# tau-dev/SdfBox

Measured on AMD Instinct MI355X. Metric: Mray/s (primary rays; frame W*H / time per frame), higher is better.
Workload: dtype f32

## Files before the change

### include/sdfhip_experimental.h

```cpp
#ifndef SDFHIP_EXPERIMENTAL_H
#define SDFHIP_EXPERIMENTAL_H

#include "sdfhip.h"

#ifdef __cplusplus
extern "C" {
#endif

enum {
    SDFHIP_FLAG_WIRE = 0x10000,
    SDFHIP_TUNE_ORDER_SHIFT = 8,
    SDFHIP_TUNE_BLOCK_SHIFT = 12,
    SDFHIP_TUNE_ONE_KERNEL = 0x20000,
    SDFHIP_TUNE_LDS_TOP = 0x40000,
    SDFHIP_TUNE_SHADOW_QUEUE = 0x80000,
    SDFHIP_TUNE_BYTE_CELLS = 0x200000,
    SDFHIP_TUNE_PERSISTENT_WAVES = 0x400000
};


SDFHIP_API int sdfhip_multi_debug_floats_sent(sdfhip_multi *m, uint32_t floats);

SDFHIP_API int sdfhip_debug_tile_order(sdfhip_scene *scene, const uint32_t *d_perm, uint16_t *d_cost);

SDFHIP_API int sdfhip_debug_touch_begin(sdfhip_scene *scene);
SDFHIP_API int sdfhip_debug_touch_end(sdfhip_scene *scene, uint64_t *out, uint32_t max_phases, uint32_t *n_phases, uint64_t *array_bytes4);

SDFHIP_API int sdfhip_debug_fail_host_allocations(int64_t countdown, uint64_t *thrown_so_far);

SDFHIP_API int sdfhip_debug_step_classes(sdfhip_scene *scene, void *stream, uint64_t *out6);

SDFHIP_API int sdfhip_debug_unorm_table(int device, float *out256);

#ifdef __cplusplus
}
#endif
#endif
```

### sdfbox_amd/_lib.py

```python
import ctypes
import os

_HERE = os.path.dirname(os.path.abspath(__file__))
LIB_PATH = os.path.abspath(os.environ.get("SDFHIP_LIB") or os.path.join(_HERE, "libsdfhip.so"))
LAB_LIB_PATH = os.path.join(_HERE, "libsdfhip_lab.so")

try:
    import torch
except Exception:
    torch = None

if not os.path.exists(LIB_PATH):
    raise ImportError(
        f"{LIB_PATH} is missing: build it with `make -C {os.path.join(_HERE, 'csrc')}` "
        "(hipcc --offload-arch=gfx950). sdfbox_amd has no CPU fallback.")

lib = ctypes.CDLL(LIB_PATH)

OK, ERR_ARG, ERR_IO, ERR_BAD_TREE, ERR_DEVICE, ERR_NOMEM = range(6)

KERNEL_AUTO, KERNEL_GENERIC, KERNEL_STACK = 0, 1, 2
FLAG_COMPACT, FLAG_COUNT, FLAG_DISPLAY, FLAG_DISPLAY_DEBUG = 0x10, 0x20, 0x40, 0x80
FLAG_TILE_ORDER = 0x100000
FLAG_WIRE = 0x10000
# ... 515 lines not shown
    "sdfhip_trimesh_prepare": (_c.c_int, [_vp, _c.c_uint32, _c.c_uint32, _c.POINTER(TriMeshOptions), _c.POINTER(CTriMesh)]),
    "sdfhip_trimesh_free": (None, [_c.POINTER(CTriMesh)]),
    "sdfhip_trimesh_build": (_c.c_int, [_c.c_int, _c.POINTER(CTriMesh), _c.c_int32, _c.POINTER(_vp), _c.POINTER(COctData),
                                        _c.POINTER(TriMeshStats)]),
    "sdfhip_scene_top_grid": (_c.c_int, [_vp, _c.POINTER(_c.c_int32), _c.POINTER(_c.c_uint64)]),
    "sdfhip_render_bands_device": (_c.c_int, [_vp, _c.POINTER(Info), _c.c_uint32, _c.POINTER(PathTrace), _c.c_uint32,
                                              _c.c_uint32, _c.c_uint32, _c.POINTER(_c.c_uint16), _c.c_uint32,
                                              _c.c_uint32, _c.c_uint32, _vp, _vp, _c.POINTER(Stats)]),
    "sdfhip_deinterleave_bands_device": (_c.c_int, [_c.c_int, _vp, _vp, _c.c_uint32, _c.c_uint32, _c.c_uint32,
                                                    _c.c_uint32, _c.c_uint32, _c.POINTER(_c.c_uint8), _c.c_uint32,
                                                    _c.c_uint32, _vp]),
    "sdfhip_sparse2_bytes": (_c.c_uint64, [_c.c_uint32, _c.c_uint32, _c.c_uint32, _c.c_uint32]),
    "sdfhip_sparse2_floats_offset": (_c.c_uint64, [_c.c_uint32, _c.c_uint32, _c.c_uint32]),
    "sdfhip_render_sparse_device": (_c.c_int, [_vp, _c.POINTER(Info), _c.c_uint32, _c.c_uint32, _c.c_uint32, _c.c_uint32,
                                               _c.POINTER(_c.c_uint16), _c.c_uint32, _c.c_uint32, _c.c_uint32, _c.c_uint32, _c.c_uint32, _vp, _vp]),
    "sdfhip_deinterleave_sparse2_device": (_c.c_int, [_c.c_int, _c.POINTER(_vp), _vp, _c.c_uint32, _c.c_uint32, _c.c_uint32,
                                                      _c.c_uint32, _c.c_uint32, _c.POINTER(_c.c_uint8), _c.c_uint32, _c.c_uint32,
                                                      _c.c_uint32, _c.c_int, _vp, _vp]),
    "sdfhip_multi_create": (_c.c_int, [_c.POINTER(_c.c_int), _c.c_uint32, _vp, _vp, _c.c_uint32, _c.POINTER(_vp)]),
    "sdfhip_multi_free": (_c.c_int, [_vp]),
    "sdfhip_multi_configure": (_c.c_int, [_vp, _c.c_uint32, _c.c_float]),
    "sdfhip_multi_info": (_c.c_int, [_vp, _c.POINTER(_c.c_uint32), _c.POINTER(_c.c_int), _c.POINTER(_c.c_uint32),
                                     _c.POINTER(_c.c_float), _c.POINTER(_c.c_int)]),
    "sdfhip_multi_render": (_c.c_int, [_vp, _c.POINTER(Info), _c.c_uint32, _c.c_uint32, _c.c_uint32, _vp, _c.POINTER(MultiStats)]),
    "sdfhip_multi_render_path": (_c.c_int, [_vp, _c.POINTER(Info), _c.POINTER(PathTrace), _c.c_uint32, _c.c_uint32, _c.c_uint32,
                                            _vp, _c.POINTER(MultiStats)]),
    "sdfhip_multi_submit": (_c.c_int, [_vp, _c.c_uint32, _c.POINTER(Info), _c.c_uint32, _c.c_uint32, _c.c_uint32, _c.c_uint32, _vp]),
    "sdfhip_multi_submit_path": (_c.c_int, [_vp, _c.c_uint32, _c.POINTER(Info), _c.POINTER(PathTrace), _c.c_uint32, _c.c_uint32,
                                            _c.c_uint32, _vp]),
    "sdfhip_multi_wait": (_c.c_int, [_vp, _c.c_uint32, _c.POINTER(_vp), _c.POINTER(MultiStats)]),
}
_SIG_LAB = {
    "sdfhip_debug_tile_order": (_c.c_int, [_vp, _vp, _vp]),
    "sdfhip_debug_unorm_table": (_c.c_int, [_c.c_int, _vp]),
    "sdfhip_debug_step_classes": (_c.c_int, [_vp, _vp, _c.POINTER(_c.c_uint64)]),
    "sdfhip_multi_debug_floats_sent": (_c.c_int, [_vp, _c.c_uint32]),
    "sdfhip_debug_fail_host_allocations": (_c.c_int, [_c.c_int64, _c.POINTER(_c.c_uint64)]),
    "sdfhip_debug_touch_begin": (_c.c_int, [_vp]),
    "sdfhip_debug_touch_end": (_c.c_int, [_vp, _c.POINTER(_c.c_uint64), _c.c_uint32, _c.POINTER(_c.c_uint32), _c.POINTER(_c.c_uint64)]),
}
for _name, (_res, _args) in _SIG.items():
    _fn = getattr(lib, _name)
    _fn.restype = _res
    _fn.argtypes = _args
EXPERIMENTS = hasattr(lib, "sdfhip_debug_unorm_table")
if EXPERIMENTS:
    for _name, (_res, _args) in _SIG_LAB.items():
        _fn = getattr(lib, _name)
        _fn.restype = _res
        _fn.argtypes = _args

EXPORTED_SYMBOLS = tuple(_SIG)
EXPERIMENTAL_SYMBOLS = tuple(_SIG_LAB)


def need_lab(what):
    if not EXPERIMENTS:
        raise RuntimeError(f"{what} is part of the experiments build (include/sdfhip_experimental.h): load libsdfhip_lab.so "
                           "(sdfbox_amd.lab.load(), or SDFHIP_LIB=sdfbox_amd/libsdfhip_lab.so)")



def check(code):
    if code != OK:
        raise SdfHipError(code, lib.sdfhip_last_error().decode("utf-8", "replace"))
```

### sdfbox_amd/csrc/lab.hip

```cpp
#ifndef SDFHIP_EXPERIMENTS
#error "lab.hip belongs to the experiments build (-DSDFHIP_EXPERIMENTS)"
#endif
#include "lab_kernels.h"
#include "scene.h"
#include "abi_guard.h"
#include "../../include/sdfhip_experimental.h"

#include <atomic>
#include <cstdlib>
#include <new>

using namespace sdfhip;

void sdfhip::build_dense4(sdfhip_scene *s)
{
    const int F = (int)s->depth;
    if (!s->stack_ok || !s->d_top || F < 1 || F > 10 || s->top_level + s->fine_bits != F) return;
    const char *env = getenv("SDFHIP_SAMPLE_RECORDS");
    if (!env || atoi(env) != 1) return;
    const size_t ncell = (size_t)1 << (3 * F);
    if (ncell * 4 > s->total_mem / 32) return;
    const GridRef g{s->d_top, s->d_fine, s->top_level, s->fine_bits, 0};
    const uint32_t n_chunks = (uint32_t)((ncell + 255) / 256);
    uint32_t *d4 = nullptr, *d_chunks = nullptr;
// ... 120 lines not shown
            if (cur == CUR_STACK_SPLIT) { if (count) go(k_path<CUR_STACK_SPLIT, true>); else go(k_path<CUR_STACK_SPLIT, false>); }
            else                        { if (count) go(k_path<CUR_STACK_FULL, true>); else go(k_path<CUR_STACK_FULL, false>); }
            *launched = true;
        }
        return SDFHIP_OK;
    }
    if (compact) return SDFHIP_OK;
    const uint32_t tile_w = bt >= 128 ? 16u : 8u, tile_h = (uint32_t)bt / 8u / (tile_w / 8u);
    P.tiles_x = (c.width + tile_w - 1) / tile_w;
    P.tiles_y = (c.nrows_out + tile_h - 1) / tile_h;
    P.n_tiles = P.tiles_x * P.tiles_y;
    const dim3 gp(P.tile_order == 0 ? 8u * ((P.tiles_y + 7u) / 8u) * P.tiles_x : P.n_tiles, c.n_frames);
    if ((flags & SDFHIP_TUNE_LDS_TOP) && cur == CUR_STACK && s->d_top && s->top_level <= 3 && !count) {
        if (bt == 256) hipLaunchKernelGGL((k_plain<CUR_STACK, false, 256, true>), gp, dim3(256), 0, st, P);
        else           hipLaunchKernelGGL((k_plain<CUR_STACK, false, 64, true>), gp, dim3(64), 0, st, P);
    }
    else if (cur == CUR_STACK_SPLIT) { if (count) launch_plain<CUR_STACK_SPLIT, true>(bt, gp, st, P); else launch_plain<CUR_STACK_SPLIT, false>(bt, gp, st, P); }
    else if (cur == CUR_STACK_FULL)  { if (count) launch_plain<CUR_STACK_FULL, true>(bt, gp, st, P); else launch_plain<CUR_STACK_FULL, false>(bt, gp, st, P); }
    else if (cur == CUR_STACK)       { if (count) launch_plain<CUR_STACK, true>(bt, gp, st, P); else launch_plain<CUR_STACK, false>(bt, gp, st, P); }
    else                             { if (count) launch_plain<CUR_GENERIC, true>(bt, gp, st, P); else launch_plain<CUR_GENERIC, false>(bt, gp, st, P); }
    *launched = true;
    return SDFHIP_OK;
}

extern "C" int sdfhip_debug_tile_order(sdfhip_scene *s, const uint32_t *d_perm, uint16_t *d_cost)
try {
    if (!s) return fail(SDFHIP_ERR_ARG, "debug_tile_order: null scene");
    std::lock_guard<std::mutex> lk(s->lock);
    s->dbg_tile_perm = d_perm; s->dbg_tile_cost = d_cost;
    return SDFHIP_OK;
}
SDFHIP_ABI_CATCH(sdfhip_debug_tile_order)

static void touch_release(sdfhip_scene *s)
{
    for (int a = 0; a < 4; a++) { if (s->touch.bits[a]) (void)hipFree(s->touch.bits[a]); s->touch.bits[a] = nullptr; s->touch.words[a] = 0; }
    if (s->touch.result) (void)hipFree(s->touch.result);
    s->touch.result = nullptr; s->touch.on = false; s->touch.phase = 0;
}

void sdfhip::touch_params(const sdfhip_scene *s, RenderParams &P, int pair)
{
    P.touch_top = s->touch.bits[pair]; P.touch_top_words = s->touch.words[pair];
    P.touch_fine = s->touch.bits[pair + 1]; P.touch_fine_words = s->touch.words[pair + 1];
}

void sdfhip::touch_phase(sdfhip_scene *s, hipStream_t st, int pair)
{
    if (!s->touch.on || s->touch.phase >= sdfhip_scene::Touch::MAX_PHASES) return;
    unsigned long long *out = s->touch.result + (size_t)s->touch.phase * 8;
    const uint32_t most = s->touch.words[pair] > s->touch.words[pair + 1] ? s->touch.words[pair] : s->touch.words[pair + 1];
    const uint32_t blocks = (most + 255u) / 256u < 4096u ? (most + 255u) / 256u : 4096u;
    hipLaunchKernelGGL(k_touch_count, dim3(blocks ? blocks : 1u), dim3(256), 0, st, s->touch.bits[pair], s->touch.words[pair],
                       s->touch.bits[pair + 1], s->touch.words[pair + 1], out);
    const unsigned long long which = (unsigned long long)pair;
    (void)hipMemcpyAsync(out + 4, &which, sizeof which, hipMemcpyHostToDevice, st);
    s->touch.phase++;
}

extern "C" int sdfhip_debug_touch_begin(sdfhip_scene *s)
try {
    if (!s) return fail(SDFHIP_ERR_ARG, "debug_touch_begin: null scene");
    std::lock_guard<std::mutex> lk(s->lock);
    DeviceGuard g(s->device);
    if (!g.ok) return (void)hipGetLastError(), fail(SDFHIP_ERR_DEVICE, "debug_touch_begin: hipSetDevice(%d) failed", s->device);
    if (!s->d_top || s->top_level + s->fine_bits != (int)s->depth)
// ... 109 lines not shown
```

### sdfbox_amd/csrc/render.hip

```cpp
#include "raymarch_kernels.h"
#include "tile_order_kernels.h"
#include "scene.h"
#include "abi_guard.h"
#ifdef SDFHIP_EXPERIMENTS
#include "../../include/sdfhip_experimental.h"
#endif

#include <chrono>
#include <cmath>
#include <cstdlib>
#include <cstring>
#include <vector>

using namespace sdfhip;

namespace {

struct Plan {
    bool use_stack = false, compact = false, count = false, grid_lookup = false;
    bool persistent = false;
    int cur = CUR_GENERIC;
    uint32_t out_mode = 0;
    dim3 grid;
    sdfhip_scene::Scratch *sc = nullptr;
};

void unpack_info(const sdfhip_info *in, FrameInfo &I)
{
    I.h0x = in->heading[0][0]; I.h0y = in->heading[0][1]; I.h0z = in->heading[0][2];
    I.h1x = in->heading[1][0]; I.h1y = in->heading[1][1]; I.h1z = in->heading[1][2];
    I.h2x = in->heading[2][0]; I.h2y = in->heading[2][1]; I.h2z = in->heading[2][2];
    I.posx = in->position[0]; I.posy = in->position[1]; I.posz = in->position[2];
    I.margin = in->margin;
    I.margin2 = in->margin * 2.0f;
    I.screen_w = in->screen_size[0]; I.screen_h = in->screen_size[1];
    I.limit = in->limit;
    I.lightx = in->light[0]; I.lighty = in->light[1]; I.lightz = in->light[2];
    I.fov = in->fov;
    I.k_strength = exp2f(in->strength) - 1.0f;
    I.half_aspect = in->screen_size[0] / in->screen_size[1] * 0.5f;
}

uint32_t sky_through_the_display_pass()
{
    auto q = [](float c) { float v = powf(c, 1.0f / 2.2f); v = v > 1.0f ? 1.0f : (v > 0.0f ? v : 0.0f); return (uint32_t)(v * 255.0f + 0.5f); };
    return q(0.005f) | (q(0.01f) << 8) | (q(0.2f) << 16);
}

int fill_params(sdfhip_scene *s, const RenderCall &c, RenderParams &P, Plan &plan)
{
    if (c.n_frames == 0 || c.n_frames > (uint32_t)MAX_BATCH)
        return fail(SDFHIP_ERR_ARG, "render: n_frames %u outside 1..%d", c.n_frames, MAX_BATCH);
    if (c.width == 0 || c.height == 0 || c.nrows_out == 0 || c.band_rows == 0 || c.band_stride == 0)
        return fail(SDFHIP_ERR_ARG, "render: zero-sized frame or band");
    if ((uint64_t)c.width * c.nrows_out > 0x7FFFFFFFull)
        return fail(SDFHIP_ERR_ARG, "render: %u x %u pixels exceed the 31-bit pixel index", c.width, c.nrows_out);
    const uint32_t flags = c.flags, kind = flags & SDFHIP_KERNEL_MASK;
// ... 71 lines not shown
    plan.cur = !plan.use_stack ? CUR_GENERIC : (s->d_top && s->fine_bits) ? CUR_STACK_SPLIT :
               (s->d_top && (uint32_t)s->top_level >= s->depth) ? CUR_STACK_FULL : CUR_STACK;
    plan.grid_lookup = plan.cur == CUR_STACK_FULL || plan.cur == CUR_STACK_SPLIT;
    plan.grid = dim3(8u * ((P.tiles_y + 7u) / 8u) * P.tiles_x, c.n_frames);
    if (plan.compact && (!plan.grid_lookup || plan.persistent) && (c.width > 65535u || c.nrows_out > 65535u))
        return fail(SDFHIP_ERR_ARG, "render: the persistent-wave compact kernel packs a pixel's x and row into 16 bits each (frame %u x %u)", c.width, c.nrows_out);
    if (c.sparse && !plan.grid_lookup)
        return fail(SDFHIP_ERR_ARG, "render_sparse: this scene has no full-depth grid (trees deeper than 12 levels or with inconsistent links render dense shares)");
    return SDFHIP_OK;
}

int need_scratch(sdfhip_scene *s, const RenderCall &c, Plan &plan)
{
    if (plan.sc) return SDFHIP_OK;
    return get_scratch(s, c.st, 0, &plan.sc);
}

template <int CUR, bool COUNT>
void launch_march(uint32_t mode, dim3 flat, hipStream_t st, const RenderParams &P)
{
    const dim3 grid = march_grid(P, flat);
    if (!COUNT && P.out_host && mode <= (uint32_t)OUT_HEAT8) {
        if (mode == OUT_RGBA32F)     hipLaunchKernelGGL((k_march<CUR, false, OUT_RGBA32F | OUT_HOST, false>), grid, dim3(64), 0, st, P);
        else if (mode == OUT_GAMMA8) hipLaunchKernelGGL((k_march<CUR, false, OUT_GAMMA8 | OUT_HOST, false>), grid, dim3(64), 0, st, P);
        else                         hipLaunchKernelGGL((k_march<CUR, false, OUT_HEAT8 | OUT_HOST, false>), grid, dim3(64), 0, st, P);
        return;
    }
    if (mode == OUT_RGBA32F)     hipLaunchKernelGGL((k_march<CUR, COUNT, OUT_RGBA32F, false>), grid, dim3(64), 0, st, P);
    else if (mode == OUT_GAMMA8) hipLaunchKernelGGL((k_march<CUR, COUNT, OUT_GAMMA8, false>), grid, dim3(64), 0, st, P);
    else if (mode == OUT_HEAT8)  hipLaunchKernelGGL((k_march<CUR, COUNT, OUT_HEAT8, false>), grid, dim3(64), 0, st, P);
    else                         hipLaunchKernelGGL((k_march<CUR, COUNT, OUT_SPARSE, false>), grid, dim3(64), 0, st, P);
}

int launch_default(sdfhip_scene *s, const RenderCall &c, RenderParams &P, Plan &plan)
{
    hipStream_t st = c.st;
    const bool ordered = (c.flags & SDFHIP_FLAG_TILE_ORDER) != 0 && P.n_tiles <= 65536u && plan.grid.x / 8u <= 65535u &&
                         plan.grid.x <= 8u * 1024u * (uint32_t)ORDER_SPAN && !P.tile_perm && !P.tile_cost;
    sdfhip_scene::Scratch *sc = nullptr;
    if (ordered) {
        int rcs = need_scratch(s, c, plan);
        if (rcs != SDFHIP_OK) return rcs;
        sc = plan.sc;
        uint32_t sig[8] = { c.width, c.height, c.nrows_out, c.band_rows, c.band_first, c.band_stride, P.n_band_list, 0u };
        for (uint32_t i = 0; i < P.n_band_list; i++) sig[7] = sig[7] * 31u + c.bands[i] + 1u;
        if (P.n_tiles > sc->ord_tiles || plan.grid.x > sc->ord_blocks) {
            HIP_TRY(hipStreamSynchronize(st));
            if (sc->ord_cost) (void)hipFree(sc->ord_cost);
            if (sc->ord_class) (void)hipFree(sc->ord_class);
            if (sc->ord_perm) (void)hipFree(sc->ord_perm);
            sc->ord_cost = nullptr; sc->ord_class = nullptr; sc->ord_perm = nullptr; sc->ord_tiles = sc->ord_blocks = 0; sc->ord_valid = false;
            HIP_TRY(device_alloc((void **)&sc->ord_cost, (size_t)MAX_BATCH * P.n_tiles * sizeof(uint16_t)));
            HIP_TRY(device_alloc((void **)&sc->ord_class, (size_t)P.n_tiles));
            HIP_TRY(device_alloc((void **)&sc->ord_perm, (size_t)plan.grid.x * sizeof(uint32_t)));
            sc->ord_tiles = P.n_tiles; sc->ord_blocks = plan.grid.x;
        }
        if (memcmp(sig, sc->ord_sig, sizeof sig) != 0) { sc->ord_valid = false; memcpy(sc->ord_sig, sig, sizeof sig); }
        P.tile_perm = sc->ord_valid ? sc->ord_perm : nullptr;
        P.perm_per_label = plan.grid.x / 8u;
        const sdfhip_info *last_info = c.info + (c.n_frames - 1u);
        P.tile_cost = (sc->ord_valid && memcmp(last_info, &sc->ord_info, sizeof(sdfhip_info)) == 0) ? nullptr : sc->ord_cost;
    }
    if (plan.cur == CUR_STACK_SPLIT) { if (plan.count) launch_march<CUR_STACK_SPLIT, true>(plan.out_mode, plan.grid, st, P); else launch_march<CUR_STACK_SPLIT, false>(plan.out_mode, plan.grid, st, P); }
    else                             { if (plan.count) launch_march<CUR_STACK_FULL, true>(plan.out_mode, plan.grid, st, P); else launch_march<CUR_STACK_FULL, false>(plan.out_mode, plan.grid, st, P); }
    const sdfhip_info *last = c.info + (c.n_frames - 1u);
    if (ordered && !(sc->ord_valid && memcmp(last, &sc->ord_info, sizeof(sdfhip_info)) == 0)) {
        sc->ord_info = *last;
        hipLaunchKernelGGL(k_tile_class, dim3((P.n_tiles + 255u) / 256u), dim3(256), 0, st, sc->ord_cost + (size_t)(c.n_frames - 1u) * P.n_tiles,
                           sc->ord_class, P.tiles_x, P.tiles_y);
        hipLaunchKernelGGL(k_tile_order, dim3(8), dim3(1024), 0, st, sc->ord_class, sc->ord_perm, P.tiles_x, P.tiles_y);
        sc->ord_valid = true;
    }
    return SDFHIP_OK;
}

template <int CUR, bool COUNT>
int launch_pt_pipeline(sdfhip_scene *s, dim3 grid, hipStream_t st, RenderParams &P)
{
    const uint32_t resident = ((uint32_t)s->cu_count * 32u + 63u) & ~63u;
    hipError_t e;
    if ((e = hipMemsetAsync(P.pt_ctl, 0, sdfhip_scene::CTL_PT_WORDS * sizeof(uint32_t), st)) != hipSuccess)
        return fail(SDFHIP_ERR_DEVICE, "render_path: hipMemsetAsync failed: %s", hipGetErrorString(e));
    hipLaunchKernelGGL((k_pt_primary<CUR, COUNT>), grid, dim3(64), 0, st, P);
#ifdef SDFHIP_EXPERIMENTS
    if (COUNT && s->touch.on) touch_phase(s, st, 0);
    uint32_t pt_sort_from = 0;
    if (const char *env = getenv("SDFHIP_PT_SORT_FROM")) pt_sort_from = (uint32_t)atoi(env);
#endif
    for (uint32_t b = 0; b <= P.pt_bounces; b++) {
        P.pt_level = b;
        if (b > 0 && (e = hipMemsetAsync(P.pt_ctl + (size_t)((b & 1u) ^ 1u) * HIT_QUEUES * 32, 0, HIT_QUEUES * 32 * sizeof(uint32_t), st)) != hipSuccess)
            return fail(SDFHIP_ERR_DEVICE, "render_path: hipMemsetAsync failed: %s", hipGetErrorString(e));
        RenderParams Pb = P;
        if (s->d_top2) {
            Pb.top = s->d_top2; Pb.top_level = s->top2_level; Pb.fine = s->d_fine2; Pb.fine_bits = s->fine2_bits; Pb.fine_order = s->fine2_order;
        }
#ifdef SDFHIP_EXPERIMENTS
        if (b < pt_sort_from) Pb.pt_sort_bits = 0;
        if (Pb.pt_sort_bits) {
            const uint32_t nkeys = 8u << (3 * Pb.pt_sort_bits);
            const dim3 sort_grid((uint32_t)s->cu_count * 4u);
            if ((e = hipMemsetAsync(Pb.pt_hist, 0, ((size_t)nkeys + 1) * sizeof(uint32_t), st)) != hipSuccess)
                return fail(SDFHIP_ERR_DEVICE, "render_path: hipMemsetAsync failed: %s", hipGetErrorString(e));
            if (s->d_top2) hipLaunchKernelGGL((k_pt_key<CUR_STACK_SPLIT>), sort_grid, dim3(PT_SORT_THREADS), 0, st, Pb);
// ... 160 lines not shown
        if (!t.h_counters) HIP_TRY(hipHostMalloc((void **)&t.h_counters, 6 * sizeof(unsigned long long), hipHostMallocDefault));
        t.counted = false; t.kernel_used = 0;
        t.in_use.store(true, std::memory_order_release);
        *out = &t;
        return SDFHIP_OK;
    }
    return fail(SDFHIP_ERR_ARG, "render: %d calls with statistics are in flight on one scene handle (at most %d at a time)", sdfhip_scene::MAX_TICKETS, sdfhip_scene::MAX_TICKETS);
}

int sdfhip::finish_stats(sdfhip_scene *s, sdfhip_scene::StatsTicket *t, sdfhip_stats *stats)
{
    DeviceGuard g(s->device);
    hipError_t e = hipEventSynchronize(t->ev1);
    memset(stats, 0, sizeof *stats);
    if (e == hipSuccess) e = hipEventElapsedTime(&stats->kernel_ms, t->ev0, t->ev1);
    stats->kernel_used = t->kernel_used;
    if (e == hipSuccess && t->counted) {
        const unsigned long long *h = t->h_counters;
        stats->n_nodes = h[0]; stats->n_samples = h[1]; stats->n_steps = h[2]; stats->n_shadow_rays = h[3];
        stats->n_loads = h[4]; stats->n_hits = h[5];
    }
    t->in_use.store(false, std::memory_order_release);
    if (e != hipSuccess) return fail(SDFHIP_ERR_DEVICE, "render: waiting for the statistics failed: %s", hipGetErrorString(e));
    return SDFHIP_OK;
}

int sdfhip::render_impl(sdfhip_scene *s, const RenderCall &c, sdfhip_scene::StatsTicket *ticket)
{
    RenderParams P;
    Plan plan;
    int rc = fill_params(s, c, P, plan);
    if (rc != SDFHIP_OK) return rc;
    hipStream_t st = c.st;
    if (plan.count) {
        rc = need_scratch(s, c, plan);
        if (rc != SDFHIP_OK) return rc;
        P.counters = reinterpret_cast<unsigned long long *>(plan.sc->ctl + sdfhip_scene::CTL_HIT_WORDS + sdfhip_scene::CTL_QUEUE_WORDS + sdfhip_scene::CTL_PT_WORDS);
        HIP_TRY(hipMemsetAsync(P.counters, 0, sdfhip_scene::CTL_COUNTER_WORDS * sizeof(uint32_t), st));
    }
    if (c.pt && plan.grid_lookup) ensure_scatter_grid(s);
#ifdef SDFHIP_EXPERIMENTS
    if (s->touch.on && plan.count) touch_params(s, P, 0);
#endif
    if (ticket) HIP_TRY(hipEventRecord(ticket->ev0, st));
    bool launched = false;
#ifdef SDFHIP_EXPERIMENTS
    rc = launch_experiment(s, c, P, plan.cur, plan.count, plan.grid, &launched, &plan.sc);
    if (rc != SDFHIP_OK) return rc;
#endif
    if (!launched) {
        if (c.pt) rc = launch_path(s, c, P, plan);
        else if (plan.grid_lookup && !plan.compact) rc = launch_default(s, c, P, plan);
        else if (plan.grid_lookup && !plan.persistent) rc = launch_compact(s, c, P, plan);
        else rc = launch_fallback(s, c, P, plan);
        if (rc != SDFHIP_OK) return rc;
    }
    HIP_TRY(hipGetLastError());
#ifdef SDFHIP_EXPERIMENTS
    if (s->touch.on && plan.count && !(c.pt && plan.grid_lookup)) touch_phase(s, st, 0);
#endif
    if (ticket) {
        ticket->kernel_used = (plan.use_stack ? SDFHIP_KERNEL_STACK : SDFHIP_KERNEL_GENERIC) | (plan.compact ? SDFHIP_FLAG_COMPACT : 0u);
        if (plan.count) {
            HIP_TRY(hipMemcpyAsync(ticket->h_counters, P.counters, 6 * sizeof(unsigned long long), hipMemcpyDeviceToHost, st));
            ticket->counted = true;
        }
// ... 298 lines not shown
```

### sdfbox_amd/csrc/scene.h

```cpp
#pragma once
#include "raymarch_device.h"
#include "sdfhip_internal.h"

#include <atomic>
#include <mutex>

struct sdfhip_scene {
    int device = 0;
    uint32_t n = 0, depth = 0;
    int stack_ok = 0;
    void *alloc = nullptr;
    sdfhip::NodeRec *nodes = nullptr;
    hipStream_t stream = nullptr;
    sdfhip::TopCell *d_top = nullptr;
    int top_level = 0;
    sdfhip::TopCell *d_fine = nullptr;
    int fine_bits = 0;
    uint64_t fine_bytes = 0;
    sdfhip::TopCell *d_top2 = nullptr, *d_fine2 = nullptr;
    int top2_level = 0, fine2_bits = 0, fine2_order = 0, scatter_tried = 0;
    int opt_scatter_grid = -1, opt_scatter_order = -1;
    uint64_t top2_bytes = 0;
    size_t total_mem = 0;
    uint32_t *d_verdict = nullptr;
    struct Scratch {
        hipStream_t stream = nullptr;
        char *hit_buf = nullptr;
        size_t records = 0;
        uint32_t *ctl = nullptr;
        uint32_t launches = 0;
        uint64_t last_use = 0;
        hipEvent_t idle = nullptr;
        char *pt_buf = nullptr;
        size_t pt_bytes = 0;
        uint16_t *band_list = nullptr;
        uint32_t band_n = 0;
        uint16_t band_host[sdfhip::MAX_BAND_LIST];
        uint16_t *ord_cost = nullptr;
        uint8_t *ord_class = nullptr;
        uint32_t *ord_perm = nullptr;
        uint32_t ord_tiles = 0, ord_blocks = 0;
        uint32_t ord_sig[8] = { 0 };
        bool ord_valid = false;
        sdfhip_info ord_info;
    };
    static constexpr int MAX_SCRATCH = 16;
    static constexpr size_t CTL_HIT_WORDS = (size_t)2 * sdfhip::MAX_BATCH * sdfhip::HIT_QUEUES * 32, CTL_QUEUE_WORDS = 8 * 32,
                            CTL_PT_WORDS = (size_t)2 * sdfhip::HIT_QUEUES * 32 + 32, CTL_COUNTER_WORDS = 32;
    static constexpr size_t CTL_BYTES = (CTL_HIT_WORDS + CTL_QUEUE_WORDS + CTL_PT_WORDS + CTL_COUNTER_WORDS) * sizeof(uint32_t);
    Scratch scratch[MAX_SCRATCH];
    int n_scratch = 0;
    uint64_t uses = 0;
    struct StatsTicket {
        hipEvent_t ev0 = nullptr, ev1 = nullptr;
        unsigned long long *h_counters = nullptr;
        std::atomic<bool> in_use{false};
        bool counted = false;
        uint32_t kernel_used = 0;
    };
    static constexpr int MAX_TICKETS = 8;
    StatsTicket tickets[MAX_TICKETS];
    float4 *d_frame = nullptr;
    size_t frame_cap = 0;
    static constexpr int HOST_BANDS = 4;
    hipStream_t band_stream[HOST_BANDS] = { nullptr, nullptr, nullptr, nullptr };
    hipEvent_t band_done[HOST_BANDS] = { nullptr, nullptr, nullptr, nullptr };
    int cu_count = 0;
#ifdef SDFHIP_EXPERIMENTS
    uint32_t *d_d4 = nullptr;
    uint4 *d_recs = nullptr;
    uint64_t d4_bytes = 0;
    const uint32_t *dbg_tile_perm = nullptr;
    uint16_t *dbg_tile_cost = nullptr;
    struct Touch {
        static constexpr uint32_t MAX_PHASES = 16;
        uint32_t *bits[4] = { nullptr, nullptr, nullptr, nullptr };
        uint32_t words[4] = { 0, 0, 0, 0 };
        unsigned long long *result = nullptr;
        uint32_t phase = 0;
        bool on = false;
    } touch;
#endif
    std::mutex lock;
};

// ... 69 lines not shown
```

### sdfbox_amd/csrc/scene.hip

```cpp
#include "upload_kernels.h"
#include "scene.h"
#include "abi_guard.h"

#include <cstddef>
#include <cstdlib>
#include <cstring>
#include <new>
#include <utility>

using namespace sdfhip;

#ifndef FULL_GRID_SHARE
#define FULL_GRID_SHARE 64
#endif
#ifndef DENSE_GRID_MAX_BYTES
#define DENSE_GRID_MAX_BYTES (512ull << 20)
#endif

extern "C" int sdfhip_device_count(int *count)
try {
    if (!count) return fail(SDFHIP_ERR_ARG, "device_count: null argument");
    *count = 0;
    HIP_TRY(hipGetDeviceCount(count));
    return SDFHIP_OK;
// ... 7 lines not shown
    HIP_TRY(hipDeviceGetPCIBusId(out, (int)len, device));
    return SDFHIP_OK;
}
SDFHIP_ABI_CATCH(sdfhip_device_pci_bus_id)

extern "C" int sdfhip_scene_free(sdfhip_scene *s)
try {
    if (!s) return SDFHIP_OK;
    {
        DeviceGuard g(s->device);
        if (s->stream) (void)hipStreamSynchronize(s->stream);
        if (s->alloc) (void)hipFree(s->alloc);
        if (s->d_verdict) (void)hipFree(s->d_verdict);
        if (s->d_top) (void)hipFree(s->d_top);
        if (s->d_fine) (void)hipFree(s->d_fine);
#ifdef SDFHIP_EXPERIMENTS
        if (s->d_d4) (void)hipFree(s->d_d4);
        for (int a = 0; a < 4; a++) if (s->touch.bits[a]) (void)hipFree(s->touch.bits[a]);
        if (s->touch.result) (void)hipFree(s->touch.result);
        if (s->d_recs) (void)hipFree(s->d_recs);
#endif
        if (s->d_top2) (void)hipFree(s->d_top2);
        if (s->d_fine2) (void)hipFree(s->d_fine2);
        for (int i = 0; i < s->n_scratch; i++) {
            if (s->scratch[i].hit_buf) (void)hipFree(s->scratch[i].hit_buf);
            if (s->scratch[i].pt_buf) (void)hipFree(s->scratch[i].pt_buf);
            if (s->scratch[i].ord_cost) (void)hipFree(s->scratch[i].ord_cost);
            if (s->scratch[i].ord_class) (void)hipFree(s->scratch[i].ord_class);
            if (s->scratch[i].ord_perm) (void)hipFree(s->scratch[i].ord_perm);
            if (s->scratch[i].ctl) (void)hipFree(s->scratch[i].ctl);
            if (s->scratch[i].idle) (void)hipEventDestroy(s->scratch[i].idle);
            if (s->scratch[i].band_list) (void)hipFree(s->scratch[i].band_list);
        }
        for (int i = 0; i < sdfhip_scene::MAX_TICKETS; i++) {
            if (s->tickets[i].ev0) (void)hipEventDestroy(s->tickets[i].ev0);
            if (s->tickets[i].ev1) (void)hipEventDestroy(s->tickets[i].ev1);
            if (s->tickets[i].h_counters) (void)hipHostFree(s->tickets[i].h_counters);
        }
        if (s->d_frame) (void)hipFree(s->d_frame);
        for (int b = 0; b < sdfhip_scene::HOST_BANDS; b++) {
            if (s->band_stream[b]) { (void)hipStreamSynchronize(s->band_stream[b]); (void)hipStreamDestroy(s->band_stream[b]); }
            if (s->band_done[b]) (void)hipEventDestroy(s->band_done[b]);
        }
        if (s->stream) (void)hipStreamDestroy(s->stream);
    }
    delete s;
    return SDFHIP_OK;
}
SDFHIP_ABI_CATCH(sdfhip_scene_free)

bool sdfhip::build_split_grid(sdfhip_scene *s, int C, int FB, int order, uint64_t max_fine_bytes, TopCell **coarse_out, TopCell **fine_out,
                             uint64_t *fine_bytes_out)
{
    const size_t ncell = (size_t)1 << (3 * C);
    const uint32_t n_chunks = (uint32_t)((ncell + 255) / 256);
    uint32_t *d_block_node = nullptr, *d_chunks = nullptr;
    TopCell *d_coarse = nullptr, *d_fine = nullptr;
    bool ok = false;
    do {
        if (device_alloc((void **)&d_coarse, ncell * sizeof(TopCell)) != hipSuccess) break;
        if (device_alloc((void **)&d_chunks, ((size_t)n_chunks + 1) * 4) != hipSuccess) break;
        const uint32_t tb = (uint32_t)((ncell + 255) / 256 < 8192 ? (ncell + 255) / 256 : 8192);
        hipLaunchKernelGGL(k_top_grid, dim3(tb), dim3(256), 0, s->stream, s->nodes, d_coarse, C, 2);
        const uint32_t cb = n_chunks < 16384u ? n_chunks : 16384u;
        hipLaunchKernelGGL(k_split_count, dim3(cb), dim3(256), 0, s->stream, d_coarse, (uint32_t)ncell, n_chunks, d_chunks);
        hipLaunchKernelGGL(k_split_scan, dim3(1), dim3(1024), 0, s->stream, d_chunks, n_chunks);
// ... 74 lines not shown
                              sdfhip_scene **out, int trusted_depth)
{
    auto choice = [](int32_t given, const char *env_name, int lo, int hi) {
        if (given >= 0) return (int)given;
        if (const char *e = lab_env(env_name)) { const int v = atoi(e); if (v >= lo && v <= hi) return v; }
        return -1;
    };
    const int opt_level = choice(opt ? opt->top_grid_level : -1, "SDFHIP_TOP_GRID_LEVEL", 0, 10);
    const int opt_split = choice(opt ? opt->top_grid_split : -1, "SDFHIP_TOP_GRID_SPLIT", 0, 8);
    if (!structs || !values || !out || n == 0)
        return fail(SDFHIP_ERR_ARG, "scene_upload: null argument or empty scene");
    *out = nullptr;
    uint32_t depth = 0;
    int consistent = 0;

    int ndev = 0;
    HIP_TRY(hipGetDeviceCount(&ndev));
    if (device < 0 || device >= ndev)
        return fail(SDFHIP_ERR_DEVICE, "scene_upload: device %d of %d does not exist", device, ndev);
    DeviceGuard g(device);
    if (!g.ok) return (void)hipGetLastError(), fail(SDFHIP_ERR_DEVICE, "scene_upload: hipSetDevice(%d) failed", device);
    hipDeviceProp_t prop;
    HIP_TRY(hipGetDeviceProperties(&prop, device));
    if (strncmp(prop.gcnArchName, "gfx950", 6) != 0)
        return fail(SDFHIP_ERR_DEVICE, "scene_upload: device %d is %s; this library carries gfx950 code only", device, prop.gcnArchName);

    sdfhip_scene *s = new (std::nothrow) sdfhip_scene();
    if (!s) return fail(SDFHIP_ERR_NOMEM, "scene_upload: out of host memory");
    s->device = device; s->n = n;
    s->total_mem = prop.totalGlobalMem;
    s->cu_count = prop.multiProcessorCount;
    s->opt_scatter_grid = opt ? opt->scatter_grid : -1;
    s->opt_scatter_order = opt ? opt->scatter_order : -1;

    void *d_s = nullptr, *d_v = nullptr;
    auto bail = [&](hipError_t e, const char *what) {
        if (d_s && !resident) (void)hipFree(d_s);
        if (d_v && !resident) (void)hipFree(d_v);
        sdfhip_scene_free(s);
        return fail(SDFHIP_ERR_DEVICE, "scene_upload: %s failed: %s", what, hipGetErrorString(e));
    };
    hipError_t e;
    const size_t bytes = (size_t)n * 8;
    if ((e = hipStreamCreateWithFlags(&s->stream, hipStreamNonBlocking)) != hipSuccess) return bail(e, "hipStreamCreate");
    if ((e = device_alloc(&s->alloc, (size_t)n * 16 + 128)) != hipSuccess) return bail(e, "device_alloc(records)");
    s->nodes = reinterpret_cast<NodeRec *>(static_cast<char *>(s->alloc) + 112);
    if ((e = device_alloc((void **)&s->d_verdict, 2 * sizeof(uint32_t))) != hipSuccess) return bail(e, "device_alloc(verdict)");
    if (resident) {
        d_s = const_cast<int32_t *>(structs); d_v = const_cast<uint8_t *>(values);
    } else {
        if ((e = device_alloc(&d_s, bytes)) != hipSuccess) return bail(e, "device_alloc(structs)");
        if ((e = device_alloc(&d_v, bytes)) != hipSuccess) return bail(e, "device_alloc(values)");
        if ((e = hipMemcpyAsync(d_s, structs, bytes, hipMemcpyHostToDevice, s->stream)) != hipSuccess) return bail(e, "hipMemcpy(structs)");
        if ((e = hipMemcpyAsync(d_v, values, bytes, hipMemcpyHostToDevice, s->stream)) != hipSuccess) return bail(e, "hipMemcpy(values)");
    }
#ifdef SDFHIP_EXPERIMENTS
    const bool trust = false;
#else
    const bool trust = resident && trusted_depth >= 0;
#endif
    if (trust) {
        consistent = 1;
        depth = (uint32_t)trusted_depth;
        s->depth = depth;
        s->stack_ok = depth <= (uint32_t)LM ? 1 : 0;
    } else {
// ... 214 lines not shown
```

Baseline: 22690.

## Enable automatic cost-driven tile ordering across frames for lone default renders

Adds an automatic tile-ordering policy. When a single dense frame renders alone on the device, the march records per-tile cost, then classifies and sorts tiles into a permutation that the next frame uses, so expensive tiles are scheduled first to reduce tail imbalance. The permutation is double-buffered and reused only while the frame signature matches. Stream queries decide whether the frame is alone. The cost is extra host queries, recording cost writes, and two small kernels on report frames, and the ordering may go stale when the camera moves.

```diff
diff --git a/include/sdfhip_experimental.h b/include/sdfhip_experimental.h
--- a/include/sdfhip_experimental.h
+++ b/include/sdfhip_experimental.h
@@ -23,6 +23,8 @@
 
 SDFHIP_API int sdfhip_debug_tile_order(sdfhip_scene *scene, const uint32_t *d_perm, uint16_t *d_cost);
 
+SDFHIP_API int sdfhip_debug_last_order(sdfhip_scene *scene, int *decision);
+
 SDFHIP_API int sdfhip_debug_touch_begin(sdfhip_scene *scene);
 SDFHIP_API int sdfhip_debug_touch_end(sdfhip_scene *scene, uint64_t *out, uint32_t max_phases, uint32_t *n_phases, uint64_t *array_bytes4);
 
diff --git a/sdfbox_amd/_lib.py b/sdfbox_amd/_lib.py
--- a/sdfbox_amd/_lib.py
+++ b/sdfbox_amd/_lib.py
@@ -571,6 +571,7 @@
 }
 _SIG_LAB = {
     "sdfhip_debug_tile_order": (_c.c_int, [_vp, _vp, _vp]),
+    "sdfhip_debug_last_order": (_c.c_int, [_vp, _c.POINTER(_c.c_int)]),
     "sdfhip_debug_unorm_table": (_c.c_int, [_c.c_int, _vp]),
     "sdfhip_debug_step_classes": (_c.c_int, [_vp, _vp, _c.POINTER(_c.c_uint64)]),
     "sdfhip_multi_debug_floats_sent": (_c.c_int, [_vp, _c.c_uint32]),
diff --git a/sdfbox_amd/csrc/lab.hip b/sdfbox_amd/csrc/lab.hip
--- a/sdfbox_amd/csrc/lab.hip
+++ b/sdfbox_amd/csrc/lab.hip
@@ -176,6 +176,15 @@
 }
 SDFHIP_ABI_CATCH(sdfhip_debug_tile_order)
 
+extern "C" int sdfhip_debug_last_order(sdfhip_scene *s, int *decision)
+try {
+    if (!s || !decision) return fail(SDFHIP_ERR_ARG, "debug_last_order: null argument");
+    std::lock_guard<std::mutex> lk(s->lock);
+    *decision = s->order.last;
+    return SDFHIP_OK;
+}
+SDFHIP_ABI_CATCH(sdfhip_debug_last_order)
+
 static void touch_release(sdfhip_scene *s)
 {
     for (int a = 0; a < 4; a++) { if (s->touch.bits[a]) (void)hipFree(s->touch.bits[a]); s->touch.bits[a] = nullptr; s->touch.words[a] = 0; }
diff --git a/sdfbox_amd/csrc/order_policy.h b/sdfbox_amd/csrc/order_policy.h
--- /dev/null
+++ b/sdfbox_amd/csrc/order_policy.h
@@ -0,0 +1,54 @@
+#pragma once
+#include <cstddef>
+#include <cstdint>
+#include <cstring>
+
+namespace sdfhip {
+
+enum OrderDecision : int {
+    ORDER_PLAIN = 0,
+    ORDER_PLAIN_REPORT = 1,
+    ORDER_ORDERED = 2,
+    ORDER_ORDERED_REPORT = 3,
+    ORDER_EXPLICIT = 4
+};
+
+constexpr uint32_t ORDER_FLAG_EXPLICIT = 0x100000u;
+constexpr uint32_t ORDER_MAX_TILES = 65536u;
+constexpr uint32_t ORDER_MAX_SLOTS = 65535u;
+constexpr uint32_t ORDER_MAX_BLOCKS = 8u * 1024u * 12u;
+constexpr int ORDER_MAX_STREAMS = 8;
+
+struct OrderShape {
+    uint32_t n_frames = 1, n_tiles = 0, blocks = 0;
+    bool sparse = false, compact = false, path = false, band_list = false;
+    bool hooked = false;
+};
+
+inline bool order_shape_ok(const OrderShape &sh)
+{
+    return sh.n_frames == 1 && !sh.sparse && !sh.compact && !sh.path && !sh.band_list && !sh.hooked && sh.n_tiles > 0 &&
+           sh.n_tiles <= ORDER_MAX_TILES && sh.blocks / 8u <= ORDER_MAX_SLOTS && sh.blocks <= ORDER_MAX_BLOCKS;
+}
+
+inline bool order_alone(const int *results, int n, bool incomplete)
+{
+    if (incomplete || n <= 0) return false;
+    for (int i = 0; i < n; i++) if (results[i] != 0) return false;
+    return true;
+}
+
+inline OrderDecision order_policy(bool enabled, uint32_t flags, const OrderShape &shape, bool alone, bool state_valid,
+                                  const uint32_t state_sig[8], const uint32_t sig[8], const void *state_camera, const void *camera,
+                                  size_t camera_bytes)
+{
+    if (flags & ORDER_FLAG_EXPLICIT) return ORDER_EXPLICIT;
+    if (!enabled || !order_shape_ok(shape) || !alone) return ORDER_PLAIN;
+    if (!state_valid || memcmp(state_sig, sig, 8 * sizeof(uint32_t)) != 0) return ORDER_PLAIN_REPORT;
+    return memcmp(state_camera, camera, camera_bytes) == 0 ? ORDER_ORDERED : ORDER_ORDERED_REPORT;
+}
+
+inline bool order_uses_state(OrderDecision d) { return d == ORDER_ORDERED || d == ORDER_ORDERED_REPORT; }
+inline bool order_makes_state(OrderDecision d) { return d == ORDER_PLAIN_REPORT || d == ORDER_ORDERED_REPORT; }
+
+}
diff --git a/sdfbox_amd/csrc/render.hip b/sdfbox_amd/csrc/render.hip
--- a/sdfbox_amd/csrc/render.hip
+++ b/sdfbox_amd/csrc/render.hip
@@ -23,6 +23,7 @@
     uint32_t out_mode = 0;
     dim3 grid;
     sdfhip_scene::Scratch *sc = nullptr;
+    bool alone = false;
 };
 
 void unpack_info(const sdfhip_info *in, FrameInfo &I)
@@ -160,6 +161,67 @@
     else                         hipLaunchKernelGGL((k_march<CUR, COUNT, OUT_SPARSE, false>), grid, dim3(64), 0, st, P);
 }
 
+static_assert(ORDER_FLAG_EXPLICIT == (uint32_t)SDFHIP_FLAG_TILE_ORDER && ORDER_MAX_BLOCKS == 8u * 1024u * (uint32_t)ORDER_SPAN,
+              "order_policy.h restates the flag's bit and k_tile_order's reach");
+
+bool frame_is_alone(sdfhip_scene *s, hipStream_t st)
+{
+    sdfhip_scene::AutoOrder &o = s->order;
+    auto ask = [](hipStream_t q) { const hipError_t e = hipStreamQuery(q); if (e == hipSuccess) return 0; (void)hipGetLastError(); return e == hipErrorNotReady ? 1 : 2; };
+    hipStreamCaptureStatus cap = hipStreamCaptureStatusNone;
+    if (hipStreamIsCapturing(st, &cap) != hipSuccess) { (void)hipGetLastError(); return false; }
+    if (cap != hipStreamCaptureStatusNone) return false;
+    int me = -1;
+    for (int i = 0; i < o.n_streams; i++) if (o.streams[i] == st) me = i;
+    if (me < 0 && o.n_streams < ORDER_MAX_STREAMS) { me = o.n_streams++; o.streams[me] = st; o.pending[me] = false; }
+    if (me < 0) {
+        for (int i = 0; i < o.n_streams; i++) {
+            if (me >= 0 && o.used[i] >= o.used[me]) continue;
+            if (o.pending[i]) {
+                const int a = ask(o.streams[i]);
+                if (a == 1) continue;
+                if (a == 2) o.valid = false;
+                o.pending[i] = false;
+            }
+            me = i;
+        }
+        if (me < 0) return false;
+        o.streams[me] = st;
+    }
+    o.used[me] = ++o.clock;
+    int results[ORDER_MAX_STREAMS], n = 0;
+    bool incomplete = false, gone[ORDER_MAX_STREAMS] = { false };
+    uint64_t below = ~0ull;
+    for (int k = 0; k < o.n_streams; k++) {
+        int pick = -1;
+        for (int i = 0; i < o.n_streams; i++) if (o.used[i] < below && (pick < 0 || o.used[i] > o.used[pick])) pick = i;
+        if (pick < 0) break;
+        below = o.used[pick];
+        if (pick != me && !o.pending[pick]) continue;
+        const int a = ask(o.streams[pick]);
+        if (a == 2) { gone[pick] = true; incomplete = true; continue; }
+        results[n++] = a;
+        if (a != 0) break;
+        o.pending[pick] = false;
+    }
+    o.pending[me] = true;
+    if (incomplete) {
+        int m = 0;
+        for (int i = 0; i < o.n_streams; i++) if (!gone[i]) { o.streams[m] = o.streams[i]; o.used[m] = o.used[i]; o.pending[m] = o.pending[i]; m++; }
+        o.n_streams = m;
+        o.valid = false;
+    }
+    return order_alone(results, n, incomplete);
+}
+
+OrderShape order_shape(const RenderCall &c, const RenderParams &P, const Plan &plan)
+{
+    OrderShape sh;
+    sh.n_frames = c.n_frames; sh.n_tiles = P.n_tiles; sh.blocks = plan.grid.x;
+    sh.sparse = c.sparse; sh.compact = plan.compact; sh.path = c.pt != nullptr; sh.band_list = c.bands != nullptr;
+    return sh;
+}
+
 int launch_default(sdfhip_scene *s, const RenderCall &c, RenderParams &P, Plan &plan)
 {
     hipStream_t st = c.st;
@@ -189,6 +251,31 @@
         const sdfhip_info *last_info = c.info + (c.n_frames - 1u);
         P.tile_cost = (sc->ord_valid && memcmp(last_info, &sc->ord_info, sizeof(sdfhip_info)) == 0) ? nullptr : sc->ord_cost;
     }
+    sdfhip_scene::AutoOrder &ao = s->order;
+    OrderDecision dec = ORDER_EXPLICIT;
+    if (!(c.flags & SDFHIP_FLAG_TILE_ORDER)) {
+        OrderShape sh = order_shape(c, P, plan);
+        sh.hooked = P.tile_perm || P.tile_cost;
+        const uint32_t sig[8] = { c.width, c.height, c.nrows_out, c.band_rows, c.band_first, c.band_stride, 0u, 0u };
+        dec = order_policy(ao.enabled, c.flags, sh, plan.alone, ao.valid, ao.sig, sig, &ao.info, c.info, sizeof(sdfhip_info));
+        if (dec == ORDER_PLAIN_REPORT) {
+            ao.valid = false;
+            if (P.n_tiles > ao.tiles || plan.grid.x > ao.blocks) {
+                if (ao.cost) (void)hipFree(ao.cost);
+                if (ao.cls) (void)hipFree(ao.cls);
+                for (int b = 0; b < 2; b++) if (ao.perm[b]) (void)hipFree(ao.perm[b]);
+                ao.cost = nullptr; ao.cls = nullptr; ao.perm[0] = ao.perm[1] = nullptr; ao.tiles = ao.blocks = 0;
+                HIP_TRY(device_alloc((void **)&ao.cost, (size_t)P.n_tiles * sizeof(uint16_t)));
+                HIP_TRY(device_alloc((void **)&ao.cls, (size_t)P.n_tiles));
+                for (int b = 0; b < 2; b++) HIP_TRY(device_alloc((void **)&ao.perm[b], (size_t)plan.grid.x * sizeof(uint32_t)));
+                ao.tiles = P.n_tiles; ao.blocks = plan.grid.x;
+            }
+            memcpy(ao.sig, sig, sizeof sig);
+        }
+        if (order_uses_state(dec)) { P.tile_perm = ao.perm[ao.cur]; P.perm_per_label = plan.grid.x / 8u; }
+        if (order_makes_state(dec)) P.tile_cost = ao.cost;
+    }
+    ao.last = dec;
     if (plan.cur == CUR_STACK_SPLIT) { if (plan.count) launch_march<CUR_STACK_SPLIT, true>(plan.out_mode, plan.grid, st, P); else launch_march<CUR_STACK_SPLIT, false>(plan.out_mode, plan.grid, st, P); }
     else                             { if (plan.count) launch_march<CUR_STACK_FULL, true>(plan.out_mode, plan.grid, st, P); else launch_march<CUR_STACK_FULL, false>(plan.out_mode, plan.grid, st, P); }
     const sdfhip_info *last = c.info + (c.n_frames - 1u);
@@ -198,6 +285,13 @@
                            sc->ord_class, P.tiles_x, P.tiles_y);
         hipLaunchKernelGGL(k_tile_order, dim3(8), dim3(1024), 0, st, sc->ord_class, sc->ord_perm, P.tiles_x, P.tiles_y);
         sc->ord_valid = true;
+    }
+    if (order_makes_state(dec)) {
+        ao.info = *c.info;
+        hipLaunchKernelGGL(k_tile_class, dim3((P.n_tiles + 255u) / 256u), dim3(256), 0, st, ao.cost, ao.cls, P.tiles_x, P.tiles_y);
+        hipLaunchKernelGGL(k_tile_order, dim3(8), dim3(1024), 0, st, ao.cls, ao.perm[ao.cur ^ 1], P.tiles_x, P.tiles_y);
+        ao.cur ^= 1;
+        ao.valid = true;
     }
     return SDFHIP_OK;
 }
@@ -424,6 +518,8 @@
     int rc = fill_params(s, c, P, plan);
     if (rc != SDFHIP_OK) return rc;
     hipStream_t st = c.st;
+    if (plan.grid_lookup && !(c.flags & SDFHIP_FLAG_TILE_ORDER) && s->order.enabled && order_shape_ok(order_shape(c, P, plan)))
+        plan.alone = frame_is_alone(s, st);
     if (plan.count) {
         rc = need_scratch(s, c, plan);
         if (rc != SDFHIP_OK) return rc;
diff --git a/sdfbox_amd/csrc/scene.h b/sdfbox_amd/csrc/scene.h
--- a/sdfbox_amd/csrc/scene.h
+++ b/sdfbox_amd/csrc/scene.h
@@ -1,6 +1,7 @@
 #pragma once
 #include "raymarch_device.h"
 #include "sdfhip_internal.h"
+#include "order_policy.h"
 
 #include <atomic>
 #include <mutex>
@@ -51,6 +52,23 @@
     Scratch scratch[MAX_SCRATCH];
     int n_scratch = 0;
     uint64_t uses = 0;
+    struct AutoOrder {
+        bool enabled = true;
+        hipStream_t streams[sdfhip::ORDER_MAX_STREAMS] = { nullptr };
+        uint64_t used[sdfhip::ORDER_MAX_STREAMS] = { 0 };
+        bool pending[sdfhip::ORDER_MAX_STREAMS] = { false };
+        int n_streams = 0;
+        uint64_t clock = 0;
+        uint16_t *cost = nullptr;
+        uint8_t *cls = nullptr;
+        uint32_t *perm[2] = { nullptr, nullptr };
+        int cur = 0;
+        uint32_t tiles = 0, blocks = 0;
+        uint32_t sig[8] = { 0 };
+        bool valid = false;
+        sdfhip_info info;
+        int last = sdfhip::ORDER_PLAIN;
+    } order;
     struct StatsTicket {
         hipEvent_t ev0 = nullptr, ev1 = nullptr;
         unsigned long long *h_counters = nullptr;
diff --git a/sdfbox_amd/csrc/scene.hip b/sdfbox_amd/csrc/scene.hip
--- a/sdfbox_amd/csrc/scene.hip
+++ b/sdfbox_amd/csrc/scene.hip
@@ -63,6 +63,9 @@
             if (s->scratch[i].idle) (void)hipEventDestroy(s->scratch[i].idle);
             if (s->scratch[i].band_list) (void)hipFree(s->scratch[i].band_list);
         }
+        if (s->order.cost) (void)hipFree(s->order.cost);
+        if (s->order.cls) (void)hipFree(s->order.cls);
+        for (int b = 0; b < 2; b++) if (s->order.perm[b]) (void)hipFree(s->order.perm[b]);
         for (int i = 0; i < sdfhip_scene::MAX_TICKETS; i++) {
             if (s->tickets[i].ev0) (void)hipEventDestroy(s->tickets[i].ev0);
             if (s->tickets[i].ev1) (void)hipEventDestroy(s->tickets[i].ev1);
@@ -203,6 +206,7 @@
     s->cu_count = prop.multiProcessorCount;
     s->opt_scatter_grid = opt ? opt->scatter_grid : -1;
     s->opt_scatter_order = opt ? opt->scatter_order : -1;
+    if (const char *e = getenv("SDFHIP_AUTO_ORDER")) s->order.enabled = atoi(e) != 0;
 
     void *d_s = nullptr, *d_v = nullptr;
     auto bail = [&](hipError_t e, const char *what) {
```

New measurement: 22620 (median of 2 runs). No clear change (-0.3%).
